# 10XGenomics/supernova

Hardware: AMD Instinct MI355X
Metric: Gk-mers/s through count+graph at k=48, 1.2B×150bp; bit-exact counts (higher is better)
Workload: dtype u64

## Files before the change

### supernova_amd/csrc/snk_local.hip

```cpp
#include <string.h>
#include <cstring>
#include <rocprim/rocprim.hpp>

#include <type_traits>

#include "snk_ctx.h"
#include "snk_common.h"
#include "snk_kernels.h"
#include "snk_graph.h"
#include "snk_stages.h"

namespace {

constexpr uint32_t NONE = 0xFFFFFFFFu;
constexpr unsigned long long NONE64 = ~0ull;
constexpr uint16_t NONE16 = 0xFFFFu;
constexpr int TB = 256;

struct chunk_src {
    const uint32_t* chunk_n;
    const uint32_t* chunk_base;
    const uint4* extra;
    const unsigned long long* region_off;
    uint32_t NB, n_extra, n_regions;
// ... 129 lines not shown
    }
#pragma unroll
    for (int q = 0; q < NPT; ++q) {
        const uint32_t i = tid + q * T;
        if (i < n) {
            khi[i] = kq[q].hi;
            klo[i] = (klo_w)(kq[q].lo >> KLS);
            if (rg.keys_r) { uint64_t* d = reinterpret_cast<uint64_t*>(rg.keys_dense + ch.base + i); d[0] = kq[q].lo; d[1] = kq[q].hi; }
        }
    }
    __syncthreads();
    for (uint32_t i = tid; i < n; i += T) {
        uint32_t slot = lhash(khi[i], (uint64_t)klo[i] << KLS) & (HT - 1);
        for (;;) {
            const uint32_t old = atomicCAS(&ht[slot], 0u, i + 1u);
            if (old == 0u) break;
            slot = (slot + 1) & (HT - 1);
        }
    }
    __syncthreads();
    const uint32_t split_mask = (1u << ch.lg) - 1u;
    uint32_t mybnd = 0;
    __shared__ uint16_t mlist[8 * T];
    __shared__ uint32_t resL[T];
    __shared__ uint32_t mcnt;
#pragma unroll
    for (int q = 0; q < NPT; ++q) {
        const uint32_t i0 = q * T;
        if (i0 >= n) break;
        const uint32_t i = i0 + tid;
        const bool act = i < n;
        snk_kmer k;
        k.hi = act ? khi[i] : 0ull;
        k.lo = act ? ((uint64_t)klo[i] << KLS) : 0ull;
        uint64_t tag = 0;
        if (GR) { tag = k.lo & 0xFFFFFFFFull; k.lo &= ~0xFFFFFFFFull; }
        const uint64_t v = myv[q];
        const uint32_t c0 = (uint32_t)(v & 0xFFu);
        uint32_t keep = 0, miss = 0, nb0 = NONE, nb1 = NONE;
        const snk_kmer kr = snk_kmer_rc<K>(k);
        for (uint32_t rem = c0; rem; rem &= rem - 1) {
            const uint32_t bit = __ffs(rem) - 1;
            const snk_kmer y = bit < 4 ? snk_kmer_succ<K>(k, bit) : snk_kmer_pred<K>(k, bit - 4);
            const snk_kmer r = bit < 4 ? snk_kmer_pred<K>(kr, 3u - bit) : snk_kmer_succ<K>(kr, 7u - bit);
            const bool rev = snk_kmer_lt(r, y);
            snk_kmer cy = rev ? r : y;
            if (GR) cy.lo |= tag;
            int32_t j = -1;
            uint32_t slot = lhash(cy.hi, cy.lo) & (HT - 1);
            for (;;) {
                const uint32_t e = ht[slot];
                if (e == 0u) break;
                if (khi[e - 1] == cy.hi && ((uint64_t)klo[e - 1] << KLS) == cy.lo) { j = (int32_t)(e - 1); break; }
                slot = (slot + 1) & (HT - 1);
            }
            if (j >= 0) {
                keep |= 1u << bit;
                if (bit < 4) nb0 = ((uint32_t)j << 1) | (rev ? 1u : 0u); else nb1 = ((uint32_t)j << 1) | (rev ? 1u : 0u);
            } else miss |= 1u << bit;
        }
        if (tid == 0) mcnt = 0;
        resL[tid] = 0;
        __syncthreads();
        uint32_t pos = snk_wave_alloc(&mcnt, (uint32_t)__popc(miss));
        if (miss) {
            for (uint32_t bit = 0; bit < 8; ++bit)
                if (miss & (1u << bit)) mlist[pos++] = (uint16_t)((tid << 3) | bit);
        }
        __syncthreads();
        const uint32_t nm = mcnt;
        constexpr int SH = K - MM;
        constexpr int PER = (SH + 3) / 4;
        for (uint32_t it0 = 0; it0 < nm; it0 += T / 4) {
            const uint32_t item = it0 + (tid >> 2), sub = tid & 3u;
            const bool on = item < nm;
            const uint32_t ent = on ? mlist[item] : 0u;
            const uint32_t th = ent >> 3, bit = ent & 7u;
            const uint32_t ni = i0 + th;
            snk_kmer kk;
            kk.hi = on ? khi[ni] : 0ull;
            kk.lo = on ? ((uint64_t)klo[ni] << KLS) : 0ull;
            uint64_t ktag = 0;
            if (GR) { ktag = kk.lo & 0xFFFFFFFFull; kk.lo &= ~0xFFFFFFFFull; }
            const int first = bit < 4 ? 1 : 0;
            uint32_t mk = 0xFFFFFFFFu;
            for (int t = 0; t < PER; ++t) {
                const int sp = (int)sub * PER + t;
                if (sp < SH) {
                    const int pp = first + sp;
                    uint64_t w;
                    if (pp == 0) w = kk.hi;
                    else if (pp < 32) w = (kk.hi << (2 * pp)) | (kk.lo >> (64 - 2 * pp));
                    else if (pp == 32) w = kk.lo;
                    else w = kk.lo << (2 * pp - 64);
                    const uint32_t key = snk_mmer_key_top<MM>(w);
                    mk = key < mk ? key : mk;
                }
            }
            { const uint32_t o = __shfl_xor(mk, 1); mk = o < mk ? o : mk; }
            { const uint32_t o = __shfl_xor(mk, 2); mk = o < mk ? o : mk; }
            if (on && sub == 0) {
                const snk_kmer y = bit < 4 ? snk_kmer_succ<K>(kk, bit) : snk_kmer_pred<K>(kk, bit - 4);
                uint64_t wn;
                if (bit < 4) {
                    constexpr int pl = K - MM;
                    wn = pl < 32 ? ((y.hi << (2 * pl)) | (y.lo >> (64 - 2 * pl))) : (pl == 32 ? y.lo : (y.lo << (2 * pl - 64)));
                } else wn = y.hi;
                const uint32_t nkey = snk_mmer_key_top<MM>(wn);
                if (nkey < mk) mk = nkey;
                const uint32_t gb = snk_bucket_of_key(mk ^ (GR ? snk_group_mix((uint32_t)ktag) : 0u), NB);
                const uint32_t db = gb - (sh.bucket_base + ch.bucket);
                bool here = ch.span == 1 ? db == 0u : (gb >= sh.bucket_base + ch.bucket && db % sh.G == 0u && db / sh.G < ch.span);
                const bool remote = sh.NBl && gb / sh.NBl != sh.me;
                if (here && ch.lg) {
                    const snk_kmer r = snk_kmer_rc<K>(y);
                    snk_kmer cn = snk_kmer_lt(r, y) ? r : y;
                    if (GR) cn.lo |= ktag;
                    uint32_t h1, h2;
                    snk_kmer_hash_count<(K > 48) || GR>(cn, &h1, &h2);
                    here = (h2 & split_mask) == ch.id;
                }
                if (here && !(do_prune & 2u)) { if (!(do_prune & 1u)) atomicOr(&resL[th], 1u << bit); }
                else atomicOr(&resL[th], (1u << bit) | (0x100u << bit) | (remote ? (0x10000u << bit) : 0u));
            }
        }
        __syncthreads();
        const uint32_t res = resL[tid];
        keep |= res & 0xFFu;
        const uint32_t pm = (res >> 8) & 0xFFu;
        __syncthreads();
        if (!act) continue;
        const uint64_t gi = ch.base + i;
        ctx_out[gi] = (uint8_t)keep;
        pend_out[gi] = (uint8_t)pm;
        if (sh.premote) sh.premote[gi] = (uint8_t)(res >> 16);
        const uint32_t cnt = (uint32_t)(v >> 8);
        count_out[gi] = cnt;
        if (spec) {
            const uint32_t sc = cnt > 0xFFFFFFu ? 0xFFFFFFu : cnt;
            if (sc < (uint32_t)BL_SPEC_LDS) atomicAdd(&shist[sc], 1u);
            else if (sc < BL_SPEC_BINS) atomicAdd(&spec[sc], 1ull);
            else spec[BL_SPEC_OVER] = 1ull;
        }
        nbr_out[gi] = (nb0 == NONE ? 0x0FFFu : nb0) | (snk_kmer_eq(k, kr) ? 0x8000u : 0u) | ((nb1 == NONE ? 0x0FFFu : nb1) << 16);
        if (pm) {
            ++mybnd;
            if (gindex) {
                snk_kmer kk;
                kk.hi = khi[i];
                kk.lo = (uint64_t)klo[i] << KLS;
                uint32_t h1, h2;
                snk_kmer_hash2(kk, &h1, &h2);
                uint64_t slot = (((uint64_t)h1 << 32) | h2) & gmask;
                const unsigned long long ent = ((unsigned long long)h1 << 32) | (unsigned long long)(gi + 1);
                if (gindex[gmask + 1] == 0ull) {
                    bool placed = false;
                    for (uint32_t tries = 0; tries < 64; ++tries) {
                        const unsigned long long old = atomicCAS(&gindex[slot], 0ull, ent);
                        if (old == 0ull) { placed = true; break; }
                        slot = (slot + 1) & gmask;
                    }
                    if (!placed) gindex[gmask + 1] = 1ull;
                }
            }
        }
    }
    snk_wave_add(&bcnt, mybnd);
    __syncthreads();
    if (tid == 0) nbnd[c] = bcnt;
}
template <int K, int CAP, int T, bool BIG, bool GR, int MM>
__global__ void __launch_bounds__(T) bl_prune_kernel(const uint4* __restrict__ desc, uint32_t NB, bl_shard sh, bl_regions rg, const uint32_t* __restrict__ biglist_in,
                                                     uint32_t nchunks, uint32_t cpw,
                                                     const snk_u128* __restrict__ keys, const uint64_t* __restrict__ vals,
                                                     uint32_t do_prune, uint8_t* __restrict__ ctx_out,
                                                     uint32_t* __restrict__ count_out, uint8_t* __restrict__ pend_out,
                                                     uint32_t* __restrict__ nbr_out, uint32_t* __restrict__ nbnd,
                                                     uint32_t* __restrict__ biglist, uint32_t* __restrict__ nbig, const uint32_t* __restrict__ n_dev,
                                                     unsigned long long* __restrict__ gindex, uint64_t gmask, unsigned long long* __restrict__ spec) {
    __shared__ uint32_t shist[BL_SPEC_LDS];
    if (spec) {
        for (int j = threadIdx.x; j < BL_SPEC_LDS; j += T) shist[j] = 0;
        __syncthreads();
    }
    if (BIG && n_dev) {
        const uint32_t nb = *n_dev;
        for (uint32_t w = blockIdx.x; w < nb; w += gridDim.x)
            bl_prune_chunk<K, CAP, T, BIG, GR, MM>(biglist_in[w], desc, NB, sh, rg, keys, vals, do_prune, ctx_out, count_out, pend_out, nbr_out, nbnd, biglist, nbig, gindex, gmask,
                                                   spec, shist);
    } else {
        for (uint32_t r = 0; r < cpw; ++r) {
            const uint32_t w = blockIdx.x * cpw + r;
            if (w >= nchunks) break;
            bl_prune_chunk<K, CAP, T, BIG, GR, MM>(BIG ? biglist_in[w] : w, desc, NB, sh, rg, keys, vals, do_prune, ctx_out, count_out, pend_out, nbr_out,
                                           nbnd, biglist, nbig, gindex, gmask, spec, shist);
        }
    }
    if (spec) {
        __syncthreads();
        uint32_t* rep = reinterpret_cast<uint32_t*>(spec + BL_SPEC_BINS) + (blockIdx.x % BL_SPEC_REPL) * BL_SPEC_LDS;
        for (int j = threadIdx.x; j < BL_SPEC_LDS; j += T)
            if (shist[j]) atomicAdd(&rep[j], shist[j]);
    }
}

__global__ void __launch_bounds__(TB) bl_index_build_kernel(const snk_u128* __restrict__ keys, const uint8_t* __restrict__ pend,
                                                            uint64_t n, unsigned long long* __restrict__ tab, uint64_t mask) {
    const uint64_t i = (uint64_t)blockIdx.x * TB + threadIdx.x;
    if (i >= n || !pend[i]) return;
    const snk_kmer k = load_key(keys, i);
    uint32_t h1, h2;
    snk_kmer_hash2(k, &h1, &h2);
    uint64_t slot = (((uint64_t)h1 << 32) | h2) & mask;
    const unsigned long long ent = ((unsigned long long)h1 << 32) | (unsigned long long)(i + 1);
    for (;;) {
        const unsigned long long old = atomicCAS(&tab[slot], 0ull, ent);
        if (old == 0ull) break;
        slot = (slot + 1) & mask;
    }
}
template <int K, bool GR>
__global__ void __launch_bounds__(TB) bl_resolve_kernel(const snk_u128* __restrict__ keys, const uint8_t* __restrict__ pend,
                                                        uint64_t n, const unsigned long long* __restrict__ tab, uint64_t mask,
                                                        uint32_t do_prune, uint8_t* __restrict__ ctx, uint32_t* __restrict__ rq,
                                                        const uint8_t* __restrict__ premote) {
    constexpr int SPAN = 8 * TB;
    __shared__ uint16_t list[SPAN];
    __shared__ uint32_t cnt;
    const uint64_t base = (uint64_t)blockIdx.x * SPAN;
    if (threadIdx.x == 0) cnt = 0;
    __syncthreads();
    {
        const uint64_t i8 = base + 8ull * threadIdx.x;
        unsigned long long w = 0;
        if (i8 + 8 <= n) w = *reinterpret_cast<const unsigned long long*>(pend + i8);
        else for (uint64_t q = i8; q < n; ++q) w |= (unsigned long long)pend[q] << (8 * (q - i8));
        if (w) {
            uint32_t m = 0;
            for (int q = 0; q < 8; ++q) if ((w >> (8 * q)) & 0xFFull) ++m;
            uint32_t pos = atomicAdd(&cnt, m);
            for (int q = 0; q < 8; ++q) if ((w >> (8 * q)) & 0xFFull) list[pos++] = (uint16_t)(8 * threadIdx.x + q);
        }
    }
    __syncthreads();
    const uint32_t m = cnt;
    for (uint32_t it = threadIdx.x; it < m; it += TB) {
        const uint64_t i = base + list[it];
        const uint32_t pm = pend[i] & (premote ? ~(uint32_t)premote[i] : 0xFFu);
        snk_kmer k = load_key(keys, i);
        uint64_t tag = 0;
        if (GR) { tag = k.lo & 0xFFFFFFFFull; k.lo &= ~0xFFFFFFFFull; }
        uint32_t c = ctx[i];
        const snk_kmer kr = snk_kmer_rc<K>(k);
        for (uint32_t rem = pm; rem; rem &= rem - 1) {
            const uint32_t bit = __ffs(rem) - 1;
            const snk_kmer y = bit < 4 ? snk_kmer_succ<K>(k, bit) : snk_kmer_pred<K>(k, bit - 4);
            const snk_kmer r = bit < 4 ? snk_kmer_pred<K>(kr, 3u - bit) : snk_kmer_succ<K>(kr, 7u - bit);
            const bool rev = snk_kmer_lt(r, y);
            snk_kmer cy = rev ? r : y;
            if (GR) cy.lo |= tag;
            uint32_t h1, h2;
            snk_kmer_hash2(cy, &h1, &h2);
            uint64_t slot = (((uint64_t)h1 << 32) | h2) & mask;
            int64_t j = -1;
            for (;;) {
                const unsigned long long e = tab[slot];
                if (e == 0ull) break;
                if ((uint32_t)(e >> 32) == h1) {
                    const uint64_t idx = (uint32_t)e - 1u;
                    if (snk_kmer_eq(load_key(keys, idx), cy)) { j = (int64_t)idx; break; }
                }
                slot = (slot + 1) & mask;
            }
            if (j >= 0) rq[2 * i + (bit >> 2)] = ((uint32_t)j << 1) | (rev ? 1u : 0u);
            else if (do_prune) c &= ~(1u << bit);
            else rq[2 * i + (bit >> 2)] = NONE;
        }
        ctx[i] = (uint8_t)c;
    }
}

struct bl_extra_pool {
    unsigned long long* cur;
    uint64_t f0, b0;
    uint64_t fcap, bcap;
};
struct bl_dist_args {
    const uint8_t* premote;
    const uint32_t* rq_idx;
    const uint16_t* rq_meta;
    const unsigned long long* node_off;
    unsigned long long my_node_off;
};
template <int K, int CAP, int T, bool BIG, bool EMIT, bool DIST, bool GR>
__global__ void __launch_bounds__(T) bl_frag_kernel(const uint4* __restrict__ desc, const uint32_t* __restrict__ biglist_in,
                                                    const snk_u128* __restrict__ keys, const uint8_t* __restrict__ ctx,
                                                    const uint8_t* __restrict__ pend, const uint32_t* __restrict__ nbr,
                                                    const uint32_t* __restrict__ rq, bl_dist_args da, uint32_t* __restrict__ nfrag,
                                                    const uint32_t* __restrict__ foff, const uint64_t* __restrict__ boff,
                                                    uint32_t* __restrict__ nk, unsigned long long* __restrict__ hl_self,
                                                    unsigned long long* __restrict__ hl_nb, uint64_t* __restrict__ bstart,
                                                    uint8_t* __restrict__ fbases, uint32_t* __restrict__ fgroup, uint32_t* __restrict__ sfrag, bl_extra_pool xp) {
    constexpr int SPT = (2 * CAP + T - 1) / T;
    typedef typename std::conditional<(K <= 48 && !GR), uint32_t, uint64_t>::type klo_w;
    constexpr int KLS = (K <= 48 && !GR) ? 32 : 0;
    __shared__ uint64_t khi[CAP];
    __shared__ klo_w klo[CAP];
    __shared__ uint16_t nbL[2 * CAP];
    typedef typename std::conditional<(CAP <= 256), uint32_t, uint64_t>::type wrec_t;
    constexpr int FB = CAP <= 256 ? 10 : 16;
    constexpr uint32_t FM = (1u << FB) - 1u;
    __shared__ uint16_t lnk[2 * CAP];
    __shared__ wrec_t wr[2 * CAP];
    constexpr bool WIDE = (uint32_t)CAP * (uint32_t)K > 65535u;
    uint16_t* foffL = nbL;
    __shared__ uint32_t frel[WIDE ? CAP : 1];
    __shared__ uint16_t hnode[CAP];
    __shared__ uint8_t ctxL[CAP], pendL[CAP], palL[CAP];
    __shared__ uint32_t fcnt, bcnt, changed;
    const int tid = threadIdx.x;
    const uint32_t c = BIG ? biglist_in[blockIdx.x] : blockIdx.x;
    const chunk_t ch = chunk_get(desc, c);
    if (ch.n == 0) return;
    if (!BIG && ch.n > (uint32_t)CAP) return;
    const uint32_t n = ch.n;
    const uint32_t c_foff = EMIT ? foff[c] : 0u;
    const uint64_t c_boff = EMIT ? boff[c] : 0ull;
    if (tid == 0) { fcnt = 0; bcnt = 0; changed = 0; }
    {
        constexpr int NPT = (CAP + T - 1) / T;
        snk_kmer kq[NPT];
        uint32_t cq[NPT], pq[NPT];
        uint32_t nq[NPT];
#pragma unroll
        for (int q = 0; q < NPT; ++q) {
            const uint32_t i = tid + q * T;
            if (i < n) {
                const uint64_t gi = ch.base + i;
                if (EMIT) kq[q] = load_key(keys, gi);
                cq[q] = ctx[gi];
                pq[q] = pend[gi];
                nq[q] = nbr[gi];
            }
        }
#pragma unroll
        for (int q = 0; q < NPT; ++q) {
            const uint32_t i = tid + q * T;
            if (i < n) {
                if (EMIT) {
                    const snk_kmer k = kq[q];
                    khi[i] = k.hi;
                    klo[i] = (klo_w)(k.lo >> KLS);
                }
                palL[i] = (uint8_t)((nq[q] >> 15) & 1u);
                ctxL[i] = (uint8_t)cq[q];
                pendL[i] = (uint8_t)pq[q];
                const uint32_t a0 = nq[q] & 0x0FFFu, a1 = (nq[q] >> 16) & 0x0FFFu;
                nbL[2 * i] = a0 == 0x0FFFu ? NONE16 : (uint16_t)a0;
                nbL[2 * i + 1] = a1 == 0x0FFFu ? NONE16 : (uint16_t)a1;
            }
        }
    }
    __syncthreads();
    uint32_t myterm = 0;
    for (uint32_t s = tid; s < 2 * n; s += T) {
        const uint32_t i = s >> 1, side = s & 1u;
        const uint32_t cc = ctxL[i];
        const uint32_t bits = side ? (cc >> 4) : (cc & 15u);
        uint16_t out = NONE16;
        if (__popc(bits) == 1) {
            const uint32_t b = __ffs(bits) - 1;
            if (!((pendL[i] >> (4 * side + b)) & 1u)) {
                const uint32_t nb = nbL[s];
                if (nb != NONE16) {
                    const uint32_t j = nb >> 1, rev = nb & 1u;
                    const uint32_t fs = side ^ 1u ^ rev;
                    const uint32_t cj = ctxL[j];
                    const uint32_t deg = fs ? __popc(cj & 0xF0u) : __popc(cj & 0x0Fu);
                    if (deg == 1 && !palL[i] && !palL[j]) out = (uint16_t)((j << 1) | fs);
                }
            }
        }
        lnk[s] = out;
        if (!EMIT) { if (out == NONE16) ++myterm; }
        else if (out == NONE16) wr[s] = (wrec_t)FM | ((wrec_t)s << (2 * FB));
        else wr[s] = (wrec_t)(out ^ 1u) | ((wrec_t)1 << FB) | ((wrec_t)(out ^ 1u) << (2 * FB));
    }
    if (!EMIT) {
        snk_wave_add(&fcnt, myterm);
        __syncthreads();
        if (tid == 0) nfrag[c] = fcnt >> 1;
        return;
    }
    __syncthreads();
    int max_rounds = 2;
    while ((1u << (max_rounds - 1)) < 2 * n) ++max_rounds;
    for (int round = 0; round < max_rounds; ++round) {
        wrec_t rr[SPT];
        bool any = false;
#pragma unroll
        for (int q = 0; q < SPT; ++q) {
            if ((uint32_t)(q * T) >= 2 * n) break;
            const uint32_t s = tid + q * T;
            if (s < 2 * n) {
                const wrec_t a0 = wr[s];
                const uint32_t n1 = (uint32_t)a0 & FM;
                rr[q] = a0;
                if (n1 != FM) {
                    const wrec_t a1 = wr[n1];
                    const uint32_t d = (((uint32_t)(a0 >> FB) & FM) + ((uint32_t)(a1 >> FB) & FM)) & FM;
                    rr[q] = (a1 & (wrec_t)FM) | ((wrec_t)d << FB) | (a1 & ((wrec_t)FM << (2 * FB)));
                    any = true;
                }
            }
        }
        __syncthreads();
#pragma unroll
        for (int q = 0; q < SPT; ++q) {
            if ((uint32_t)(q * T) >= 2 * n) break;
            const uint32_t s = tid + q * T;
            if (s < 2 * n) wr[s] = rr[q];
        }
        if (any) changed = 1;
        __syncthreads();
        const bool go = changed != 0;
        __syncthreads();
        if (tid == 0) changed = 0;
        if (!go) break;
    }
    __syncthreads();
    auto w_next = [&](uint32_t st) -> uint32_t { return (uint32_t)wr[st] & FM; };
    auto w_dist = [&](uint32_t st) -> uint32_t { return (uint32_t)(wr[st] >> FB) & FM; };
    auto w_tail = [&](uint32_t st) -> uint32_t { return (uint32_t)(wr[st] >> (2 * FB)) & FM; };

    auto half_link = [&](uint32_t s) -> unsigned long long {
        const uint32_t i = s >> 1, side = s & 1u;
        const uint32_t cc = ctxL[i];
        const uint32_t bits = side ? (cc >> 4) : (cc & 15u);
        if (__popc(bits) != 1 || palL[i]) return NONE64;
        const uint32_t b = __ffs(bits) - 1;
        if (!((pendL[i] >> (4 * side + b)) & 1u)) return NONE64;
        snk_kmer k;
        k.hi = khi[i];
        k.lo = GR ? ((uint64_t)klo[i] & ~0xFFFFFFFFull) : ((uint64_t)klo[i] << KLS);
        const snk_kmer y = side ? snk_kmer_pred<K>(k, b) : snk_kmer_succ<K>(k, b);
        if (snk_kmer_eq(y, snk_kmer_rc<K>(y))) return NONE64;
        const uint64_t gi = ch.base + i;
        if (DIST && ((da.premote[gi] >> (4 * side + b)) & 1u)) {
            const uint32_t a = da.rq_idx[2 * gi + side];
            if (a == NONE) return NONE64;
            const uint32_t meta = da.rq_meta[2 * gi + side];
            const uint32_t fs = side ^ 1u ^ (meta >> 15);
            return 2ull * (da.node_off[meta & 0x7FFFu] + a) + fs;
        }
        const uint32_t a = rq[2 * gi + side];
        if (a == NONE) return NONE64;
        const uint32_t rev = a & 1u, fs = side ^ 1u ^ rev;
        return 2ull * ((DIST ? da.my_node_off : 0ull) + (a >> 1)) + fs;
    };
    auto describe = [&](uint32_t pid, uint32_t other, uint32_t cnt, bool with_half, uint32_t head_node, bool head_rc) {
        const uint32_t lf = atomicAdd(&fcnt, 1u);
        const uint32_t rel = atomicAdd(&bcnt, cnt + (uint32_t)K - 1u);
        const uint64_t f = (uint64_t)c_foff + lf;
        nk[f] = cnt;
        hl_self[2 * f] = 2ull * ((DIST ? da.my_node_off : 0ull) + ch.base) + pid;
        hl_self[2 * f + 1] = 2ull * ((DIST ? da.my_node_off : 0ull) + ch.base) + other;
        hl_nb[2 * f] = with_half ? half_link(pid) : NONE64;
        hl_nb[2 * f + 1] = with_half ? half_link(other) : NONE64;
        bstart[f] = c_boff + rel;
        if (sfrag) { sfrag[2 * ch.base + pid] = (uint32_t)(2 * f); sfrag[2 * ch.base + other] = (uint32_t)(2 * f + 1); }
        if (GR) fgroup[f] = (uint32_t)klo[head_node];
        if (WIDE) { foffL[pid] = (uint16_t)lf; frel[lf] = rel; }
        else foffL[pid] = (uint16_t)rel;
        hnode[lf] = (uint16_t)((head_node << 1) | (head_rc ? 1u : 0u));
        return rel;
    };

    for (uint32_t i = tid; i < n; i += T) {
        if (w_next(2 * i) != FM) continue;
        const uint32_t tR = w_tail(2 * i), tL = w_tail(2 * i + 1), dR = w_dist(2 * i), dL = w_dist(2 * i + 1);
        const bool fwd = tL < tR;
        const uint32_t pos = fwd ? dL : dR;
        if (pos == 0) describe(fwd ? tL : tR, fwd ? tR : tL, dR + dL + 1u, true, i, !fwd);
    }
    for (uint32_t i = tid; i < n; i += T) {
        if (w_next(2 * i) == FM) continue;
        uint32_t cur = i << 1, mn = i, cnt = 1;
        bool closed = false;
        while (cnt <= n) {
            const uint32_t l = lnk[cur];
            if (l == NONE16) break;
            const uint32_t j = l >> 1;
            if (j == i) { closed = true; break; }
            if (khi[j] < khi[mn] || (khi[j] == khi[mn] && klo[j] < klo[mn])) mn = j;
            cur = l ^ 1u;
            ++cnt;
        }
        if (closed && mn == i) {
            const unsigned long long xf = atomicAdd(&xp.cur[0], 1ull);
            const unsigned long long xb = atomicAdd(&xp.cur[1], (unsigned long long)(cnt + K - 1));
            if (xf < xp.fcap && xb + cnt + K - 1 <= xp.bcap) {
                uint32_t e = i << 1;
                for (uint32_t q = 1; q < cnt; ++q) e = lnk[e] ^ 1u;
                const uint64_t f = xp.f0 + xf, bo = xp.b0 + xb;
                const uint32_t pid = (i << 1) | 1u;
                nk[f] = cnt;
                hl_self[2 * f] = 2ull * ((DIST ? da.my_node_off : 0ull) + ch.base) + pid;
                hl_self[2 * f + 1] = 2ull * ((DIST ? da.my_node_off : 0ull) + ch.base) + e;
                hl_nb[2 * f] = NONE64;
                hl_nb[2 * f + 1] = NONE64;
                bstart[f] = bo;
                if (sfrag) { sfrag[2 * ch.base + pid] = (uint32_t)(2 * f); sfrag[2 * ch.base + e] = (uint32_t)(2 * f + 1); }
                if (GR) fgroup[f] = (uint32_t)klo[i];
                snk_kmer k;
                k.hi = khi[i];
                k.lo = (uint64_t)klo[i] << KLS;
                for (int b = 0; b < K; ++b) fbases[bo + b] = (uint8_t)oriented_base<K>(k, false, b);
                uint32_t curs = i << 1;
                for (uint32_t pos = 1; pos < cnt; ++pos) {
                    const uint32_t l = lnk[curs];
                    k.hi = khi[l >> 1];
                    k.lo = (uint64_t)klo[l >> 1] << KLS;
                    fbases[bo + (K - 1) + pos] = (uint8_t)oriented_base<K>(k, (l & 1u) == 0, K - 1);
                    curs = l ^ 1u;
                }
            }
        }
    }
    __syncthreads();
    for (uint32_t i = tid; i < n; i += T) {
        if (w_next(2 * i) != FM) continue;
        const uint32_t tR = w_tail(2 * i), tL = w_tail(2 * i + 1), dR = w_dist(2 * i), dL = w_dist(2 * i + 1);
        const bool fwd = tL < tR;
        const uint32_t pos = fwd ? dL : dR;
        if (pos == 0) continue;
        snk_kmer k;
        k.hi = khi[i];
        k.lo = (uint64_t)klo[i] << KLS;
        const uint32_t fo = foffL[fwd ? tL : tR];
        fbases[c_boff + (WIDE ? frel[fo] : fo) + (K - 1) + pos] = (uint8_t)oriented_base<K>(k, !fwd, K - 1);
    }
    struct __attribute__((packed)) u32_any { uint32_t v; };
    const uint32_t nheads = fcnt;
    constexpr int HPI = T / 16;
    static_assert(K % 4 == 0 && K / 4 <= 16, "a head is K / 4 dwords, one per lane of its group");
    for (uint32_t h0 = 0; h0 < nheads; h0 += HPI) {
        const uint32_t h = h0 + (tid >> 4);
        const int q = tid & 15;
        if (h < nheads && q < K / 4) {
            const uint32_t hn = hnode[h];
            const uint32_t i = hn >> 1;
            const bool rc = hn & 1u;
            uint32_t fo;
            if (WIDE) fo = frel[h];
            else { const uint32_t tR = w_tail(2 * i), tL = w_tail(2 * i + 1); fo = foffL[tL < tR ? tL : tR]; }
            snk_kmer k;
            k.hi = khi[i];
            k.lo = (uint64_t)klo[i] << KLS;
            const uint32_t v = oriented_base<K>(k, rc, 4 * q) | (oriented_base<K>(k, rc, 4 * q + 1) << 8) | (oriented_base<K>(k, rc, 4 * q + 2) << 16) |
                               (oriented_base<K>(k, rc, 4 * q + 3) << 24);
            reinterpret_cast<u32_any*>(fbases + c_boff + fo + 4 * q)->v = v;
        }
    }
}

__global__ void __launch_bounds__(TB) bl_chunk_bases_kernel(const uint4* __restrict__ desc, const uint32_t* __restrict__ nfrag, uint32_t nchunks,
                                                            uint32_t K, uint64_t* __restrict__ nbases) {
    const uint32_t c = blockIdx.x * TB + threadIdx.x;
    if (c > nchunks) return;
    if (c == nchunks) { nbases[c] = 0; return; }
    const uint32_t n = desc[c].y;
    nbases[c] = nfrag[c] ? (uint64_t)n + (uint64_t)(K - 1) * nfrag[c] : 0ull;
}

__global__ void __launch_bounds__(TB) bl_pack_vals_kernel(const uint32_t* __restrict__ counts, const uint8_t* __restrict__ ctx,
                                                          uint64_t n, uint64_t* __restrict__ vals) {
    const uint64_t i = (uint64_t)blockIdx.x * TB + threadIdx.x;
    if (i < n) vals[i] = ((uint64_t)counts[i] << 8) | ctx[i];
}
__global__ void __launch_bounds__(TB) bl_unpack_vals_kernel(const uint64_t* __restrict__ vals, uint64_t n,
                                                            uint32_t* __restrict__ counts, uint8_t* __restrict__ ctx) {
    const uint64_t i = (uint64_t)blockIdx.x * TB + threadIdx.x;
    if (i < n) { counts[i] = (uint32_t)(vals[i] >> 8); ctx[i] = (uint8_t)(vals[i] & 0xFFu); }
}

}

#define G_ALLOC(ptr, type, count)                                                       \
    do {                                                                                \
        void* _p = nullptr;                                                             \
        int _rc = snk_ctx_alloc(ctx, sizeof(type) * (size_t)(count), &_p, err, errcap); \
        if (_rc) return _rc;                                                            \
        ptr = (type*)_p;                                                                \
    } while (0)

template <typename T>
static int excl_scan(snk_ctx* ctx, hipStream_t st, const T* in, T* out, size_t count, char* err, size_t errcap) {
    size_t tb = 0;
    SNK_HIP_TRY(rocprim::exclusive_scan((void*)nullptr, tb, in, out, (T)0, count, rocprim::plus<T>(), st));
    void* tmp;
    int rc = snk_ctx_alloc(ctx, tb, &tmp, err, errcap);
    if (rc) return rc;
    SNK_HIP_TRY(rocprim::exclusive_scan(tmp, tb, in, out, (T)0, count, rocprim::plus<T>(), st));
    return SNK_OK;
}

constexpr int SCAP = 256, ST = 64;
constexpr int BCAP = SNK_GRAPH_CHUNK_MAX, BT = 256;

namespace {
constexpr int QWORDS = 4;
constexpr int QSPAN = 8 * QWORDS * TB;
template <int K, bool FILL>
__global__ void __launch_bounds__(TB) bl_query_kernel(const snk_u128* __restrict__ keys, const uint8_t* __restrict__ premote, uint64_t n,
                                                      uint32_t NB_total, uint32_t NBl, uint32_t world, uint32_t mlen,
                                                      unsigned long long* __restrict__ qcount_or_cursor,
                                                      unsigned long long* __restrict__ qbuf) {
    extern __shared__ unsigned long long dynq[];
    __shared__ uint16_t list[QSPAN];
    __shared__ uint32_t cnt;
    uint32_t* lcur = reinterpret_cast<uint32_t*>(dynq + world);
    const uint64_t base = (uint64_t)blockIdx.x * QSPAN;
    if (threadIdx.x == 0) cnt = 0;
    for (uint32_t r = threadIdx.x; r < world; r += TB) { dynq[r] = 0; lcur[r] = 0; }
    __syncthreads();
    for (int t = 0; t < QWORDS; ++t) {
        const uint32_t w0 = 8u * ((uint32_t)t * TB + threadIdx.x);
        const uint64_t i8 = base + w0;
        unsigned long long w = 0;
        if (i8 + 8 <= n) w = *reinterpret_cast<const unsigned long long*>(premote + i8);
        else for (uint64_t q = i8; q < n; ++q) w |= (unsigned long long)premote[q] << (8 * (q - i8));
        if (w) {
            uint32_t m = 0;
            for (int q = 0; q < 8; ++q) if ((w >> (8 * q)) & 0xFFull) ++m;
            uint32_t pos = atomicAdd(&cnt, m);
            for (int q = 0; q < 8; ++q) if ((w >> (8 * q)) & 0xFFull) list[pos++] = (uint16_t)(w0 + q);
        }
    }
    __syncthreads();
    const uint32_t m = cnt;
    for (uint32_t it = threadIdx.x; it < m; it += TB) {
        const uint64_t i = base + list[it];
        const snk_kmer k = load_key(keys, i);
        for (uint32_t rem = premote[i]; rem; rem &= rem - 1) {
            const uint32_t bit = __ffs(rem) - 1;
            const snk_kmer y = bit < 4 ? snk_kmer_succ<K>(k, bit) : snk_kmer_pred<K>(k, bit - 4);
            const uint32_t owner = (mlen == (uint32_t)SNK_M_LONG ? snk_bucket_of_kmer<K, SNK_M_LONG>(y, NB_total) : snk_bucket_of_kmer<K, SNK_M_OF(K)>(y, NB_total)) / NBl;
            atomicAdd(&dynq[owner], 1ull);
        }
    }
    __syncthreads();
    for (uint32_t r = threadIdx.x; r < world; r += TB) {
        const unsigned long long c = dynq[r];
        if (c) dynq[r] = FILL ? atomicAdd(&qcount_or_cursor[r], c) : (atomicAdd(&qcount_or_cursor[r], c), 0ull);
    }
    if (!FILL) return;
    __syncthreads();
    for (uint32_t it = threadIdx.x; it < m; it += TB) {
        const uint64_t i = base + list[it];
        const snk_kmer k = load_key(keys, i);
        for (uint32_t rem = premote[i]; rem; rem &= rem - 1) {
            const uint32_t bit = __ffs(rem) - 1;
            const snk_kmer y = bit < 4 ? snk_kmer_succ<K>(k, bit) : snk_kmer_pred<K>(k, bit - 4);
            const uint32_t owner = (mlen == (uint32_t)SNK_M_LONG ? snk_bucket_of_kmer<K, SNK_M_LONG>(y, NB_total) : snk_bucket_of_kmer<K, SNK_M_OF(K)>(y, NB_total)) / NBl;
            const snk_kmer r = snk_kmer_rc<K>(y);
            const bool rev = snk_kmer_lt(r, y);
            const snk_kmer c = rev ? r : y;
            const unsigned long long slot = dynq[owner] + atomicAdd(&lcur[owner], 1u);
            qbuf[3 * slot + 0] = c.lo;
            qbuf[3 * slot + 1] = c.hi;
            qbuf[3 * slot + 2] = (unsigned long long)i | ((unsigned long long)bit << 32) | ((unsigned long long)(rev ? 1 : 0) << 40);
        }
    }
}
}

template <int K, bool GR>
static int bl_prune_impl(snk_ctx* ctx, hipStream_t st, snk_bl_state* B, char* err, size_t errcap) {
    const snk_table* tab = B->tab;
    const uint64_t n = tab->n;
    chunk_src cs;
    cs.chunk_n = tab->chunk_n;
    cs.chunk_base = tab->chunk_base;
    cs.extra = tab->extra;
    cs.region_off = tab->region_off;
    cs.NB = tab->NB;
    cs.n_extra = tab->n_extra;
    cs.n_regions = tab->n_regions;
    cs.span = nullptr;
    const uint32_t merge_cap = snk_opt_is_set(ctx, SNK_OPT_chunk_merge) ? std::min<uint32_t>(snk_opt_u32(ctx, SNK_OPT_chunk_merge), (uint32_t)SCAP) : (uint32_t)SCAP;
    if (merge_cap && tab->chunk_n && tab->NB > tab->n_regions) {
        uint8_t* span;
        uint32_t* merged;
        G_ALLOC(span, uint8_t, (uint64_t)tab->NB + 1);
        G_ALLOC(merged, uint32_t, (uint64_t)tab->NB + 1);
        SNK_HIP_TRY(snk_launch(bl_chunk_merge_kernel, snk_blocks(tab->n_regions, 256), 256, 0, st, tab->chunk_n, tab->chunk_base, tab->NB, tab->n_regions, merge_cap, span, merged));
        cs.span = span;
        cs.chunk_n = merged;
    }
    const uint32_t nchunks = tab->NB + tab->n_extra;
    B->nchunks = nchunks;
    G_ALLOC(B->desc, uint4, (uint64_t)nchunks + 1);
    uint64_t* desc_src = nullptr;
    if (tab->keys_r) G_ALLOC(desc_src, uint64_t, (uint64_t)nchunks + 1);
    SNK_HIP_TRY(snk_launch(bl_chunk_desc_kernel, snk_blocks(nchunks, 256), 256, 0, st, cs, nchunks, B->desc, tab->region_cap, desc_src));
    uint32_t *nbnd, *ctr;
    G_ALLOC(B->ctx, uint8_t, n + 16);
    G_ALLOC(B->pend, uint8_t, n + 16);
    G_ALLOC(B->counts, uint32_t, n + 4);
    G_ALLOC(B->nbr, uint32_t, n + 2);
    G_ALLOC(B->rq, uint32_t, 2 * n + 2);
    G_ALLOC(nbnd, uint32_t, (uint64_t)nchunks + 1);
    G_ALLOC(B->biglist, uint32_t, n / SCAP + 2);
    G_ALLOC(ctr, uint32_t, 16);
    B->premote = nullptr;
    if (B->world > 1 || B->force_dist) {
        G_ALLOC(B->premote, uint8_t, n + 16);
        SNK_HIP_TRY(hipMemsetAsync(B->premote, 0, n + 16, st));
    }
    SNK_HIP_TRY(hipMemsetAsync(nbnd, 0, ((uint64_t)nchunks + 1) * 4, st));
    SNK_HIP_TRY(hipMemsetAsync(ctr, 0, 64, st));
    bl_shard sh;
    sh.bucket_base = B->premote ? B->rank * B->NBl : 0u;
    sh.NBl = B->premote ? B->NBl : 0u;
    sh.me = B->rank;
    sh.G = tab->n_regions ? tab->n_regions : 1u;
    sh.premote = B->premote;
    const uint32_t NBh = B->premote ? B->NB_total : tab->NB;
    const uint32_t cpw = snk_opt_u32(ctx, SNK_OPT_bl_cpw);
    uint64_t tg0 = 0;
    unsigned long long* index0 = nullptr;
    if (snk_opt_u32(ctx, SNK_OPT_bl_index_fused)) {
        const uint64_t guess = (ctx->last_bnd_n == n && ctx->last_bnd) ? ctx->last_bnd + ctx->last_bnd / 8 : n / 5;
        tg0 = 1024;
        while (tg0 < 2 * guess) tg0 <<= 1;
        G_ALLOC(index0, unsigned long long, tg0 + 1);
        SNK_HIP_TRY(hipMemsetAsync(index0, 0, (tg0 + 1) * 8, st));
    }
    unsigned long long* spec = nullptr;
    if (B->want_spec) {
        G_ALLOC(spec, unsigned long long, BL_SPEC_WORDS);
        SNK_HIP_TRY(hipMemsetAsync(spec, 0, (size_t)BL_SPEC_WORDS * 8, st));
    }
    bl_regions rg;
    rg.keys_r = tab->keys_r; rg.vals_r = tab->vals_r; rg.desc_src = desc_src;
    rg.keys_dense = const_cast<snk_u128*>(tab->keys);
    const bool long_m = ctx->mlen == (uint32_t)SNK_M_LONG;
    SNK_HIP_TRY(snk_launch(long_m ? bl_prune_kernel<K, SCAP, ST, false, GR, SNK_M_LONG> : bl_prune_kernel<K, SCAP, ST, false, GR, SNK_M_OF(K)>, snk_blocks(nchunks, cpw), ST, 0, st, (const uint4*)B->desc, NBh, sh, rg,
                           (const uint32_t*)nullptr, nchunks, cpw, tab->keys, tab->vals, B->do_prune | (snk_opt_u32(ctx, SNK_OPT_bl_noclassify) ? 2u : 0u), B->ctx, B->counts, B->pend, B->nbr, nbnd,
                           B->biglist, ctr, (const uint32_t*)nullptr, index0, tg0 - 1, spec));
    uint32_t h_nbig = 0;
    SNK_HIP_TRY(hipMemcpyAsync(ctr + 1, ctr, 4, hipMemcpyDeviceToDevice, st));
    SNK_HIP_TRY(snk_launch(long_m ? bl_prune_kernel<K, BCAP, BT, true, GR, SNK_M_LONG> : bl_prune_kernel<K, BCAP, BT, true, GR, SNK_M_OF(K)>, 2048, BT, 0, st, (const uint4*)B->desc, NBh, sh, rg,
                           (const uint32_t*)B->biglist, 0u, 1u, tab->keys, tab->vals, B->do_prune | (snk_opt_u32(ctx, SNK_OPT_bl_noclassify) ? 2u : 0u), B->ctx, B->counts, B->pend, B->nbr,
                           nbnd, B->biglist, ctr + 2, (const uint32_t*)(ctr + 1), index0, tg0 - 1, spec));
    if (spec) SNK_HIP_TRY(snk_launch(bl_spec_fold_kernel, 1, BL_SPEC_LDS, 0, st, spec));
    if (tab->keys_r) {
        snk_ctx_release_block(ctx, tab->keys_r);
        snk_ctx_release_block(ctx, tab->vals_r);
    }
    unsigned long long* d_sum;
    G_ALLOC(d_sum, unsigned long long, 2);
    {
        size_t tb = 0;
        auto in = rocprim::make_transform_iterator(nbnd, [] __device__(uint32_t v) { return (unsigned long long)v; });
        SNK_HIP_TRY(rocprim::reduce((void*)nullptr, tb, in, d_sum, 0ull, (size_t)nchunks, rocprim::plus<unsigned long long>(), st));
        void* tmp;
        int rc = snk_ctx_alloc(ctx, tb, &tmp, err, errcap);
        if (rc) return rc;
        SNK_HIP_TRY(rocprim::reduce(tmp, tb, in, d_sum, 0ull, (size_t)nchunks, rocprim::plus<unsigned long long>(), st));
    }
    unsigned long long h_bnd = 0, h_gaveup = 0, h_spec_over = 0;
    if (index0) SNK_HIP_TRY(hipMemcpyAsync(&h_gaveup, index0 + tg0, 8, hipMemcpyDeviceToHost, st));
    if (spec) SNK_HIP_TRY(hipMemcpyAsync(&h_spec_over, spec + BL_SPEC_OVER, 8, hipMemcpyDeviceToHost, st));
    SNK_HIP_TRY(hipMemcpyAsync(&h_bnd, d_sum, 8, hipMemcpyDeviceToHost, st));
    SNK_HIP_TRY(hipMemcpyAsync(&h_nbig, ctr + 1, 4, hipMemcpyDeviceToHost, st));
    SNK_HIP_TRY(snk_sync(st));
    B->nbig = h_nbig;
    B->spec = spec;
    B->spec_over = h_spec_over != 0;
    B->n_boundary = h_bnd;
    ctx->last_bnd = h_bnd; ctx->last_bnd_n = n;
    uint64_t tg = 1024;
    while (tg < 2 * h_bnd) tg <<= 1;
    const bool fused_ok = index0 && !h_gaveup && h_bnd * 4 <= tg0 * 3;
    if (fused_ok) { B->index = index0; tg = tg0; }
    else {
        if (index0) snk_ctx_release_block(ctx, index0);
        G_ALLOC(B->index, unsigned long long, tg);
        SNK_HIP_TRY(hipMemsetAsync(B->index, 0, tg * 8, st));
    }
    B->index_mask = tg - 1;
    if (h_bnd) {
        if (!fused_ok) SNK_HIP_TRY(snk_launch(bl_index_build_kernel, snk_blocks(n, TB), TB, 0, st, tab->keys, B->pend, n, B->index, tg - 1));
        SNK_HIP_TRY(snk_launch(bl_resolve_kernel<K, GR>, snk_blocks(n, 8 * TB), TB, 0, st, tab->keys, B->pend, n,
                               B->index, tg - 1, B->do_prune, B->ctx, B->rq, (const uint8_t*)B->premote));
    }
    return SNK_OK;
}

template <int K, bool DIST, bool GR>
static int bl_fragments_impl(snk_ctx* ctx, hipStream_t st, snk_bl_state* B, const bl_dist_args& da, snk_frag_out* out, char* err,
                             size_t errcap) {
    const snk_table* tab = B->tab;
    const uint32_t nchunks = B->nchunks, h_nbig = B->nbig;
    uint32_t *nfrag, *foff;
    uint64_t *nbases, *boff;
    G_ALLOC(nfrag, uint32_t, (uint64_t)nchunks + 1);
    G_ALLOC(foff, uint32_t, (uint64_t)nchunks + 1);
    G_ALLOC(nbases, uint64_t, (uint64_t)nchunks + 1);
    G_ALLOC(boff, uint64_t, (uint64_t)nchunks + 1);
    SNK_HIP_TRY(hipMemsetAsync(nfrag, 0, ((uint64_t)nchunks + 1) * 4, st));
    bl_extra_pool xp0;
    memset(&xp0, 0, sizeof xp0);
    SNK_HIP_TRY(snk_launch(bl_frag_kernel<K, SCAP, ST, false, false, DIST, GR>, nchunks, ST, 0, st, (const uint4*)B->desc,
                           (const uint32_t*)nullptr, tab->keys, B->ctx, B->pend, B->nbr, B->rq, da, nfrag, (const uint32_t*)nullptr,
                           (const uint64_t*)nullptr, (uint32_t*)nullptr, (unsigned long long*)nullptr, (unsigned long long*)nullptr,
                           (uint64_t*)nullptr, (uint8_t*)nullptr, (uint32_t*)nullptr, (uint32_t*)nullptr, xp0));
    SNK_HIP_TRY(snk_launch(bl_frag_kernel<K, BCAP, BT, true, false, DIST, GR>, h_nbig, BT, 0, st, (const uint4*)B->desc,
                           (const uint32_t*)B->biglist, tab->keys, B->ctx, B->pend, B->nbr, B->rq, da, nfrag, (const uint32_t*)nullptr,
                           (const uint64_t*)nullptr, (uint32_t*)nullptr, (unsigned long long*)nullptr, (unsigned long long*)nullptr,
                           (uint64_t*)nullptr, (uint8_t*)nullptr, (uint32_t*)nullptr, (uint32_t*)nullptr, xp0));
    SNK_HIP_TRY(snk_launch(bl_chunk_bases_kernel, snk_blocks((uint64_t)nchunks + 1, TB), TB, 0, st, (const uint4*)B->desc, nfrag, nchunks,
                           (uint32_t)K, nbases));
    int rc;
    if ((rc = excl_scan<uint32_t>(ctx, st, nfrag, foff, (size_t)nchunks + 1, err, errcap))) return rc;
    if ((rc = excl_scan<uint64_t>(ctx, st, nbases, boff, (size_t)nchunks + 1, err, errcap))) return rc;
    uint32_t h_F = 0;
    uint64_t h_B = 0;
    SNK_HIP_TRY(hipMemcpyAsync(&h_F, foff + nchunks, 4, hipMemcpyDeviceToHost, st));
    SNK_HIP_TRY(hipMemcpyAsync(&h_B, boff + nchunks, 8, hipMemcpyDeviceToHost, st));
    SNK_HIP_TRY(snk_sync(st));
    unsigned long long* xcur;
    G_ALLOC(xcur, unsigned long long, 2);
    const uint32_t pool0 = snk_opt_u32(ctx, SNK_OPT_bl_pool);
    uint64_t xf_cap = pool0 ? pool0 + h_F / 256 : 0, xb_cap = xf_cap * (K + 63);
    unsigned long long h_x[2] = {0, 0};
    for (int attempt = 0; attempt < 2; ++attempt) {
        ctx->last_bl_attempts = (uint32_t)attempt + 1;
        G_ALLOC(out->nk, uint32_t, (uint64_t)h_F + xf_cap + 1);
        G_ALLOC(out->hl_self, unsigned long long, 2ull * (h_F + xf_cap) + 2);
        G_ALLOC(out->hl_nb, unsigned long long, 2ull * (h_F + xf_cap) + 2);
        G_ALLOC(out->boff, uint64_t, (uint64_t)h_F + xf_cap + 2);
        G_ALLOC(out->bases, uint8_t, h_B + xb_cap + 16);
        out->fgroup = nullptr;
        if (GR) G_ALLOC(out->fgroup, uint32_t, (uint64_t)h_F + xf_cap + 1);
        G_ALLOC(out->sfrag, uint32_t, 2 * tab->n + 2);
        SNK_HIP_TRY(hipMemsetAsync(xcur, 0, 16, st));
        bl_extra_pool xp;
        xp.cur = xcur;
        xp.f0 = h_F;
        xp.b0 = h_B;
        xp.fcap = xf_cap;
        xp.bcap = xb_cap;
        SNK_HIP_TRY(snk_launch(bl_frag_kernel<K, SCAP, ST, false, true, DIST, GR>, nchunks, ST, 0, st, (const uint4*)B->desc,
                               (const uint32_t*)nullptr, tab->keys, B->ctx, B->pend, B->nbr, B->rq, da, nfrag, foff, boff, out->nk, out->hl_self,
                               out->hl_nb, out->boff, out->bases, out->fgroup, out->sfrag, xp));
        SNK_HIP_TRY(snk_launch(bl_frag_kernel<K, BCAP, BT, true, true, DIST, GR>, h_nbig, BT, 0, st, (const uint4*)B->desc,
                               (const uint32_t*)B->biglist, tab->keys, B->ctx, B->pend, B->nbr, B->rq, da, nfrag, foff, boff, out->nk,
                               out->hl_self, out->hl_nb, out->boff, out->bases, out->fgroup, out->sfrag, xp));
        SNK_HIP_TRY(hipMemcpyAsync(h_x, xcur, 16, hipMemcpyDeviceToHost, st));
// ... 179 lines not shown
```

Before: 99.54.

## Specialize fragment kernel for single-wave blocks with register keys and wave scans

Adds a single-wavefront (T==64) path to the fragment kernel. Keys stay in registers and are fetched with shuffles or reloaded from global memory instead of being staged in shared memory. Head allocation uses ballot/scan rather than shared atomics, and pointer jumping exits early via __any, which removes a barrier. The palindrome flag is packed into the neighbor word, and cycle detection now stops at the first smaller key instead of tracking a minimum. The aim is lower LDS use for higher occupancy and fewer atomics and barriers, paid for with extra global key reloads and more register pressure.

```diff
diff --git a/supernova_amd/csrc/snk_local.hip b/supernova_amd/csrc/snk_local.hip
--- a/supernova_amd/csrc/snk_local.hip
+++ b/supernova_amd/csrc/snk_local.hip
@@ -455,10 +455,12 @@
                                                     unsigned long long* __restrict__ hl_nb, uint64_t* __restrict__ bstart,
                                                     uint8_t* __restrict__ fbases, uint32_t* __restrict__ fgroup, uint32_t* __restrict__ sfrag, bl_extra_pool xp) {
     constexpr int SPT = (2 * CAP + T - 1) / T;
+    constexpr int NPT = (CAP + T - 1) / T;
+    constexpr bool ONEW = T == 64;
     typedef typename std::conditional<(K <= 48 && !GR), uint32_t, uint64_t>::type klo_w;
     constexpr int KLS = (K <= 48 && !GR) ? 32 : 0;
-    __shared__ uint64_t khi[CAP];
-    __shared__ klo_w klo[CAP];
+    __shared__ uint64_t khi[ONEW ? 1 : CAP];
+    __shared__ klo_w klo[ONEW ? 1 : CAP];
     __shared__ uint16_t nbL[2 * CAP];
     typedef typename std::conditional<(CAP <= 256), uint32_t, uint64_t>::type wrec_t;
     constexpr int FB = CAP <= 256 ? 10 : 16;
@@ -469,7 +471,7 @@
     uint16_t* foffL = nbL;
     __shared__ uint32_t frel[WIDE ? CAP : 1];
     __shared__ uint16_t hnode[CAP];
-    __shared__ uint8_t ctxL[CAP], pendL[CAP], palL[CAP];
+    __shared__ uint8_t ctxL[CAP], pendL[CAP];
     __shared__ uint32_t fcnt, bcnt, changed;
     const int tid = threadIdx.x;
     const uint32_t c = BIG ? biglist_in[blockIdx.x] : blockIdx.x;
@@ -479,10 +481,12 @@
     const uint32_t n = ch.n;
     const uint32_t c_foff = EMIT ? foff[c] : 0u;
     const uint64_t c_boff = EMIT ? boff[c] : 0ull;
-    if (tid == 0) { fcnt = 0; bcnt = 0; changed = 0; }
+    if constexpr (!ONEW) {
+        if (tid == 0) { fcnt = 0; bcnt = 0; changed = 0; }
+    }
+    uint32_t w_frags = 0, w_bases = 0;
+    snk_kmer kq[NPT] = {};
     {
-        constexpr int NPT = (CAP + T - 1) / T;
-        snk_kmer kq[NPT];
         uint32_t cq[NPT], pq[NPT];
         uint32_t nq[NPT];
 #pragma unroll
@@ -500,21 +504,35 @@
         for (int q = 0; q < NPT; ++q) {
             const uint32_t i = tid + q * T;
             if (i < n) {
-                if (EMIT) {
+                if constexpr (EMIT && !ONEW) {
                     const snk_kmer k = kq[q];
                     khi[i] = k.hi;
                     klo[i] = (klo_w)(k.lo >> KLS);
                 }
-                palL[i] = (uint8_t)((nq[q] >> 15) & 1u);
                 ctxL[i] = (uint8_t)cq[q];
                 pendL[i] = (uint8_t)pq[q];
-                const uint32_t a0 = nq[q] & 0x0FFFu, a1 = (nq[q] >> 16) & 0x0FFFu;
-                nbL[2 * i] = a0 == 0x0FFFu ? NONE16 : (uint16_t)a0;
-                nbL[2 * i + 1] = a1 == 0x0FFFu ? NONE16 : (uint16_t)a1;
+                nbL[2 * i] = (uint16_t)(nq[q] & 0x8FFFu);
+                nbL[2 * i + 1] = (uint16_t)((nq[q] >> 16) & 0x0FFFu);
             }
         }
     }
     __syncthreads();
+    auto is_pal = [&](uint32_t i) -> bool { return (nbL[2 * i] >> 15) != 0; };
+    auto key_of = [&](uint32_t i) -> snk_kmer {
+        snk_kmer k;
+        if constexpr (ONEW) {
+            k = load_key(keys, ch.base + i);
+            k.lo = (k.lo >> KLS) << KLS;
+        } else {
+            k.hi = khi[i];
+            k.lo = (uint64_t)klo[i] << KLS;
+        }
+        return k;
+    };
+    auto own_key = [&](int q, uint32_t i) -> snk_kmer {
+        if constexpr (ONEW) return kq[q];
+        else return key_of(i);
+    };
     uint32_t myterm = 0;
     for (uint32_t s = tid; s < 2 * n; s += T) {
         const uint32_t i = s >> 1, side = s & 1u;
@@ -524,13 +542,13 @@
         if (__popc(bits) == 1) {
             const uint32_t b = __ffs(bits) - 1;
             if (!((pendL[i] >> (4 * side + b)) & 1u)) {
-                const uint32_t nb = nbL[s];
-                if (nb != NONE16) {
+                const uint32_t nb = nbL[s] & 0x0FFFu;
+                if (nb != 0x0FFFu) {
                     const uint32_t j = nb >> 1, rev = nb & 1u;
                     const uint32_t fs = side ^ 1u ^ rev;
                     const uint32_t cj = ctxL[j];
                     const uint32_t deg = fs ? __popc(cj & 0xF0u) : __popc(cj & 0x0Fu);
-                    if (deg == 1 && !palL[i] && !palL[j]) out = (uint16_t)((j << 1) | fs);
+                    if (deg == 1 && !is_pal(i) && !is_pal(j)) out = (uint16_t)((j << 1) | fs);
                 }
             }
         }
@@ -540,9 +558,14 @@
         else wr[s] = (wrec_t)(out ^ 1u) | ((wrec_t)1 << FB) | ((wrec_t)(out ^ 1u) << (2 * FB));
     }
     if (!EMIT) {
-        snk_wave_add(&fcnt, myterm);
-        __syncthreads();
-        if (tid == 0) nfrag[c] = fcnt >> 1;
+        if constexpr (ONEW) {
+            const uint32_t total = (uint32_t)__builtin_amdgcn_readlane((int)snk_wave_scan_incl(myterm), 63);
+            if (tid == 0) nfrag[c] = total >> 1;
+        } else {
+            snk_wave_add(&fcnt, myterm);
+            __syncthreads();
+            if (tid == 0) nfrag[c] = fcnt >> 1;
+        }
         return;
     }
     __syncthreads();
@@ -567,6 +590,9 @@
                 }
             }
         }
+        if constexpr (ONEW) {
+            if (!__any(any)) break;
+        }
         __syncthreads();
 #pragma unroll
         for (int q = 0; q < SPT; ++q) {
@@ -574,12 +600,16 @@
             const uint32_t s = tid + q * T;
             if (s < 2 * n) wr[s] = rr[q];
         }
-        if (any) changed = 1;
-        __syncthreads();
-        const bool go = changed != 0;
-        __syncthreads();
-        if (tid == 0) changed = 0;
-        if (!go) break;
+        if constexpr (ONEW) {
+            __syncthreads();
+        } else {
+            if (any) changed = 1;
+            __syncthreads();
+            const bool go = changed != 0;
+            __syncthreads();
+            if (tid == 0) changed = 0;
+            if (!go) break;
+        }
     }
     __syncthreads();
     auto w_next = [&](uint32_t st) -> uint32_t { return (uint32_t)wr[st] & FM; };
@@ -590,12 +620,11 @@
         const uint32_t i = s >> 1, side = s & 1u;
         const uint32_t cc = ctxL[i];
         const uint32_t bits = side ? (cc >> 4) : (cc & 15u);
-        if (__popc(bits) != 1 || palL[i]) return NONE64;
+        if (__popc(bits) != 1 || is_pal(i)) return NONE64;
         const uint32_t b = __ffs(bits) - 1;
         if (!((pendL[i] >> (4 * side + b)) & 1u)) return NONE64;
-        snk_kmer k;
-        k.hi = khi[i];
-        k.lo = GR ? ((uint64_t)klo[i] & ~0xFFFFFFFFull) : ((uint64_t)klo[i] << KLS);
+        snk_kmer k = key_of(i);
+        if (GR) k.lo &= ~0xFFFFFFFFull;
         const snk_kmer y = side ? snk_kmer_pred<K>(k, b) : snk_kmer_succ<K>(k, b);
         if (snk_kmer_eq(y, snk_kmer_rc<K>(y))) return NONE64;
         const uint64_t gi = ch.base + i;
@@ -611,45 +640,65 @@
         const uint32_t rev = a & 1u, fs = side ^ 1u ^ rev;
         return 2ull * ((DIST ? da.my_node_off : 0ull) + (a >> 1)) + fs;
     };
-    auto describe = [&](uint32_t pid, uint32_t other, uint32_t cnt, bool with_half, uint32_t head_node, bool head_rc) {
-        const uint32_t lf = atomicAdd(&fcnt, 1u);
-        const uint32_t rel = atomicAdd(&bcnt, cnt + (uint32_t)K - 1u);
+    auto describe = [&](uint32_t lf, uint32_t rel, uint32_t pid, uint32_t other, uint32_t cnt, uint32_t head_node, bool head_rc, uint32_t group) {
         const uint64_t f = (uint64_t)c_foff + lf;
         nk[f] = cnt;
         hl_self[2 * f] = 2ull * ((DIST ? da.my_node_off : 0ull) + ch.base) + pid;
         hl_self[2 * f + 1] = 2ull * ((DIST ? da.my_node_off : 0ull) + ch.base) + other;
-        hl_nb[2 * f] = with_half ? half_link(pid) : NONE64;
-        hl_nb[2 * f + 1] = with_half ? half_link(other) : NONE64;
+        hl_nb[2 * f] = half_link(pid);
+        hl_nb[2 * f + 1] = half_link(other);
         bstart[f] = c_boff + rel;
         if (sfrag) { sfrag[2 * ch.base + pid] = (uint32_t)(2 * f); sfrag[2 * ch.base + other] = (uint32_t)(2 * f + 1); }
-        if (GR) fgroup[f] = (uint32_t)klo[head_node];
-        if (WIDE) { foffL[pid] = (uint16_t)lf; frel[lf] = rel; }
+        if (GR) fgroup[f] = group;
+        if constexpr (WIDE) { foffL[pid] = (uint16_t)lf; frel[lf] = rel; }
         else foffL[pid] = (uint16_t)rel;
         hnode[lf] = (uint16_t)((head_node << 1) | (head_rc ? 1u : 0u));
-        return rel;
     };
 
-    for (uint32_t i = tid; i < n; i += T) {
-        if (w_next(2 * i) != FM) continue;
-        const uint32_t tR = w_tail(2 * i), tL = w_tail(2 * i + 1), dR = w_dist(2 * i), dL = w_dist(2 * i + 1);
-        const bool fwd = tL < tR;
-        const uint32_t pos = fwd ? dL : dR;
-        if (pos == 0) describe(fwd ? tL : tR, fwd ? tR : tL, dR + dL + 1u, true, i, !fwd);
+#pragma unroll
+    for (int q = 0; q < NPT; ++q) {
+        if ((uint32_t)(q * T) >= n) break;
+        const uint32_t i = tid + q * T;
+        bool head = false, fwd = false;
+        uint32_t tR = 0, tL = 0, cnt = 0;
+        if (i < n && w_next(2 * i) == FM) {
+            tR = w_tail(2 * i); tL = w_tail(2 * i + 1);
+            const uint32_t dR = w_dist(2 * i), dL = w_dist(2 * i + 1);
+            fwd = tL < tR;
+            head = (fwd ? dL : dR) == 0;
+            cnt = dR + dL + 1u;
+        }
+        const uint32_t nb = head ? cnt + (uint32_t)K - 1u : 0u;
+        uint32_t lf = 0, rel = 0;
+        if constexpr (ONEW) {
+            const unsigned long long hm = __ballot(head);
+            if (hm == 0) continue;
+            const uint32_t incl = snk_wave_scan_incl(nb);
+            lf = w_frags + (uint32_t)__popcll(hm & ((1ull << tid) - 1ull));
+            rel = w_bases + incl - nb;
+            w_frags += (uint32_t)__popcll(hm);
+            w_bases += (uint32_t)__builtin_amdgcn_readlane((int)incl, 63);
+        } else if (head) {
+            lf = atomicAdd(&fcnt, 1u);
+            rel = atomicAdd(&bcnt, nb);
+        }
+        if (head) describe(lf, rel, fwd ? tL : tR, fwd ? tR : tL, cnt, i, !fwd, GR ? (uint32_t)own_key(q, i).lo : 0u);
     }
     for (uint32_t i = tid; i < n; i += T) {
         if (w_next(2 * i) == FM) continue;
-        uint32_t cur = i << 1, mn = i, cnt = 1;
+        uint32_t cur = i << 1, cnt = 1;
+        const snk_kmer ki = key_of(i);
         bool closed = false;
         while (cnt <= n) {
             const uint32_t l = lnk[cur];
             if (l == NONE16) break;
             const uint32_t j = l >> 1;
             if (j == i) { closed = true; break; }
-            if (khi[j] < khi[mn] || (khi[j] == khi[mn] && klo[j] < klo[mn])) mn = j;
+            if (snk_kmer_lt(key_of(j), ki)) break;
             cur = l ^ 1u;
             ++cnt;
         }
-        if (closed && mn == i) {
+        if (closed) {
             const unsigned long long xf = atomicAdd(&xp.cur[0], 1ull);
             const unsigned long long xb = atomicAdd(&xp.cur[1], (unsigned long long)(cnt + K - 1));
             if (xf < xp.fcap && xb + cnt + K - 1 <= xp.bcap) {
@@ -664,16 +713,13 @@
                 hl_nb[2 * f + 1] = NONE64;
                 bstart[f] = bo;
                 if (sfrag) { sfrag[2 * ch.base + pid] = (uint32_t)(2 * f); sfrag[2 * ch.base + e] = (uint32_t)(2 * f + 1); }
-                if (GR) fgroup[f] = (uint32_t)klo[i];
-                snk_kmer k;
-                k.hi = khi[i];
-                k.lo = (uint64_t)klo[i] << KLS;
+                if (GR) fgroup[f] = (uint32_t)ki.lo;
+                snk_kmer k = ki;
                 for (int b = 0; b < K; ++b) fbases[bo + b] = (uint8_t)oriented_base<K>(k, false, b);
                 uint32_t curs = i << 1;
                 for (uint32_t pos = 1; pos < cnt; ++pos) {
                     const uint32_t l = lnk[curs];
-                    k.hi = khi[l >> 1];
-                    k.lo = (uint64_t)klo[l >> 1] << KLS;
+                    k = key_of(l >> 1);
                     fbases[bo + (K - 1) + pos] = (uint8_t)oriented_base<K>(k, (l & 1u) == 0, K - 1);
                     curs = l ^ 1u;
                 }
@@ -681,35 +727,51 @@
         }
     }
     __syncthreads();
-    for (uint32_t i = tid; i < n; i += T) {
-        if (w_next(2 * i) != FM) continue;
+#pragma unroll
+    for (int q = 0; q < NPT; ++q) {
+        const uint32_t i = tid + q * T;
+        if (i >= n || w_next(2 * i) != FM) continue;
         const uint32_t tR = w_tail(2 * i), tL = w_tail(2 * i + 1), dR = w_dist(2 * i), dL = w_dist(2 * i + 1);
         const bool fwd = tL < tR;
         const uint32_t pos = fwd ? dL : dR;
         if (pos == 0) continue;
-        snk_kmer k;
-        k.hi = khi[i];
-        k.lo = (uint64_t)klo[i] << KLS;
-        const uint32_t fo = foffL[fwd ? tL : tR];
-        fbases[c_boff + (WIDE ? frel[fo] : fo) + (K - 1) + pos] = (uint8_t)oriented_base<K>(k, !fwd, K - 1);
+        const snk_kmer k = own_key(q, i);
+        uint32_t fo = foffL[fwd ? tL : tR];
+        if constexpr (WIDE) fo = frel[fo];
+        fbases[c_boff + fo + (K - 1) + pos] = (uint8_t)oriented_base<K>(k, !fwd, K - 1);
     }
     struct __attribute__((packed)) u32_any { uint32_t v; };
-    const uint32_t nheads = fcnt;
+    uint32_t nheads = w_frags;
+    if constexpr (!ONEW) nheads = fcnt;
     constexpr int HPI = T / 16;
     static_assert(K % 4 == 0 && K / 4 <= 16, "a head is K / 4 dwords, one per lane of its group");
     for (uint32_t h0 = 0; h0 < nheads; h0 += HPI) {
         const uint32_t h = h0 + (tid >> 4);
         const int q = tid & 15;
-        if (h < nheads && q < K / 4) {
-            const uint32_t hn = hnode[h];
-            const uint32_t i = hn >> 1;
-            const bool rc = hn & 1u;
+        const bool act = h < nheads && q < K / 4;
+        const uint32_t hn = act ? hnode[h] : 0u;
+        const uint32_t i = hn >> 1;
+        const bool rc = hn & 1u;
+        snk_kmer k;
+        if constexpr (ONEW) {
+            k.hi = 0; k.lo = 0;
+#pragma unroll
+            for (int s = 0; s < NPT; ++s) {
+                if ((uint32_t)(s * T) >= n) break;
+                const int src = (int)(i & 63u);
+                const uint32_t a0 = (uint32_t)__shfl((int)(uint32_t)(kq[s].hi >> 32), src), a1 = (uint32_t)__shfl((int)(uint32_t)kq[s].hi, src);
+                const uint32_t a2 = (uint32_t)__shfl((int)(uint32_t)(kq[s].lo >> 32), src);
+                uint32_t a3 = 0;
+                if constexpr (K > 48) a3 = (uint32_t)__shfl((int)(uint32_t)kq[s].lo, src);
+                if ((i >> 6) == (uint32_t)s) { k.hi = ((uint64_t)a0 << 32) | a1; k.lo = ((uint64_t)a2 << 32) | a3; }
+            }
+        } else {
+            k = key_of(i);
+        }
+        if (act) {
             uint32_t fo;
-            if (WIDE) fo = frel[h];
+            if constexpr (WIDE) fo = frel[h];
             else { const uint32_t tR = w_tail(2 * i), tL = w_tail(2 * i + 1); fo = foffL[tL < tR ? tL : tR]; }
-            snk_kmer k;
-            k.hi = khi[i];
-            k.lo = (uint64_t)klo[i] << KLS;
             const uint32_t v = oriented_base<K>(k, rc, 4 * q) | (oriented_base<K>(k, rc, 4 * q + 1) << 8) | (oriented_base<K>(k, rc, 4 * q + 2) << 16) |
                                (oriented_base<K>(k, rc, 4 * q + 3) << 24);
             reinterpret_cast<u32_any*>(fbases + c_boff + fo + 4 * q)->v = v;
```

New measurement: 100.7 (median of 6 runs). +1.2%, better.
